# tensor4all/tensor4all-rs

Hardware: AMD Instinct MI355X
Metric: TCI2 full-sweep GF/s (d=30, chi=256 fp64) (higher is better)
Workload: dtype f64

## Files before the change

include/t4a_gpu.h:

```cpp
#ifndef T4A_GPU_H
#define T4A_GPU_H

#include <stddef.h>
#include <stdint.h>

#ifdef __cplusplus
extern "C" {
#endif
#if defined(__GNUC__)
#pragma GCC visibility push(default)
#endif

typedef int32_t t4a_gpu_status;
#define T4A_GPU_SUCCESS 0
#define T4A_GPU_NULL_POINTER (-1)
#define T4A_GPU_INVALID_ARGUMENT (-2)
#define T4A_GPU_BUFFER_TOO_SMALL (-5)
#define T4A_GPU_INTERNAL_ERROR (-6)
#define T4A_GPU_NOT_IMPLEMENTED (-7)
#define T4A_GPU_NAN_ENCOUNTERED (-8)
#define T4A_GPU_SINGULAR_MATRIX (-9)
#define T4A_GPU_NO_DEVICE (-10)
#define T4A_GPU_KERNEL_TIMEOUT (-11)
#define T4A_GPU_CALLBACK_ERROR (-12)
// ... 559 lines not shown
                                                const double* const* col_frames, size_t row_count, size_t col_count, int32_t op_kind,
                                                t4a_gpu_aci_op_fn op, void* user, size_t max_bond_dim, double tolerance,
                                                int32_t scale_tolerance, int32_t left_orthogonal, size_t* rank, size_t* row_indices,
                                                size_t* col_indices, double* pivot_errors, size_t* n_pivot_errors, double* left,
                                                double* right, double* sampled_scale, double* local_values);

t4a_gpu_status t4a_gpu_tci2_last_sweep_shapes(const t4a_gpu_tci2* h, size_t* out);
#define T4A_GPU_PROFILE_SLOTS 16
t4a_gpu_status t4a_gpu_tci2_profile_enable(t4a_gpu_tci2* h, int32_t enable);
t4a_gpu_status t4a_gpu_tci2_profile_reset(t4a_gpu_tci2* h);
t4a_gpu_status t4a_gpu_tci2_profile_get(const t4a_gpu_tci2* h, double* out );
t4a_gpu_status t4a_gpu_tci2_profile_variants(const t4a_gpu_tci2* h, double* out , size_t cap_rows, size_t* n_rows);

t4a_gpu_status t4a_gpu_tci2_chain_stats(const t4a_gpu_tci2* h, uint64_t* out );
t4a_gpu_status t4a_gpu_tci2_chain_stats_ext(const t4a_gpu_tci2* h, uint64_t* out );
t4a_gpu_status t4a_gpu_tci2_fill_stats(const t4a_gpu_tci2* h, uint64_t* out );
t4a_gpu_status t4a_gpu_tci2_rook_stats(const t4a_gpu_tci2* h, uint64_t* out );
t4a_gpu_status t4a_gpu_tci2_optimize_group(t4a_gpu_tci2* const* handles, size_t n_handles, const t4a_gpu_tci2_options* options,
                                           int32_t final_sweep1site);
t4a_gpu_status t4a_gpu_tci2_fill_site_tensors_group(t4a_gpu_tci2* const* handles, size_t n_handles);
t4a_gpu_status t4a_gpu_tci2_set_chain(t4a_gpu_tci2* h, int32_t enable, int32_t verify);
t4a_gpu_status t4a_gpu_tci2_set_callback_threads(t4a_gpu_tci2* h, size_t n_threads);
t4a_gpu_status t4a_gpu_tci2_small_stats(const t4a_gpu_tci2* h, uint64_t* out );

t4a_gpu_status t4a_gpu_fn_eval(int32_t fid, int32_t n_acc, const double* params, const uint64_t* weights,
                               const size_t* local_dims, size_t n_sites, const size_t* idx, size_t n_pts,
                               double* out);

#define T4A_GPU_GMRES_RELATIVE 0
#define T4A_GPU_GMRES_ABSOLUTE 1
// ... 234 lines not shown
```

tensor4all-rs_amd/csrc/capi.hip:

```cpp
#include "stdrng.hpp"
#include "smallrng.hpp"
#include <memory>
#include <initializer_list>
#include <mutex>

#include "patching.hpp"
#include "tci2.hpp"
#include "tree.hpp"
#include "quantics.hpp"
#include "tensorops.hpp"
#include "dense.hpp"
#include "aci.hpp"
#include "globalsearch.hpp"
#include "mpo.hpp"
#include "contraction.hpp"
#include "quanticstransform.hpp"
#include "tt_canonical.hpp"
#include "dmrg.hpp"
#include "tdvp.hpp"
#include "gse.hpp"
#include "pmpo.hpp"
#include "linsolve.hpp"
#include "swap.hpp"

// ... 1212 lines not shown
t4a_gpu_status t4a_gpu_tci2_chain_stats(const t4a_gpu_tci2* h, uint64_t* out)
{
    return guarded([&] {
        T4A_REQUIRE_PTR(h);
        T4A_REQUIRE_PTR(out);
        for (int k = 0; k < 5; ++k) out[k] = h->impl.chain_stats[k];
    });
}

t4a_gpu_status t4a_gpu_tci2_chain_stats_ext(const t4a_gpu_tci2* h, uint64_t* out)
{
    return guarded([&] {
        T4A_REQUIRE_PTR(h);
        T4A_REQUIRE_PTR(out);
        for (int k = 0; k < 4; ++k) out[k] = h->impl.chain_stats_ext[k];
    });
}

t4a_gpu_status t4a_gpu_tci2_rook_stats(const t4a_gpu_tci2* h, uint64_t* out)
{
    return guarded([&] {
        T4A_REQUIRE_PTR(h);
        T4A_REQUIRE_PTR(out);
        const RookWork& w = h->impl.rook_work();
        out[0] = w.n_device_searches;
        out[1] = w.n_device_visits;
        out[2] = w.n_host_searches;
        out[3] = w.n_host_syncs;
    });
}
// ... 4426 lines not shown
```

tensor4all-rs_amd/csrc/kernels.hpp:

```cpp
#pragma once

#include <hip/hip_runtime.h>

#include <cstddef>
#include <cstdint>

#include "../../include/t4a_testfunctions.h"

namespace t4a {

struct RrluWorkspace;

struct RrluPlan {
    int W = 1;
    int T = 256;
    int cpw = 0;
    int Mld = 0;
    size_t lds_bytes = 0;
};

RrluPlan rrlu_make_plan(int M, int N, int num_cus);

struct RrluArgs {
    const double* A;
// ... 239 lines not shown
    const int* prev_colperm;
    unsigned prev_token;
    unsigned long long* dbg;
    int defer_host_writes;
};
struct ChainWalkArgs {
    char* blocks;
    size_t block_bytes, off_piv, off_rp, off_cp, off_ts;
    double* pi;
    int n_bonds;
    int max_steps;
    double rel_tol, abs_tol;
    double* factors;
    size_t factors_stride;
    unsigned token_base;
    int timed;
    int lean_prep;
    unsigned long long* phase_ticks;
};
void chain_walk_launch(const ChainCommon& c, const FnDevice& fn, const ChainWalkArgs& w, int columns, hipStream_t stream);
void chain_indep_launch(const ChainCommon& c, int n_bonds, hipStream_t stream);
void chain_last_core_launch(const ChainCommon& c, const FnDevice& fn, double* core, int max_entries, hipStream_t stream);
void chain_prep_launch(const ChainCommon& c, const ChainPrepArgs& a, hipStream_t stream);
void chain_pi_launch(const ChainCommon& c, const FnDevice& fn, int b, int n_dep_ub, int n_ind_ub, double* out, hipStream_t stream);

constexpr int CHAIN_GROUP_MAX = 8;
struct ChainGroupSlot {
    ChainCommon c;
    FnDevice fn;
    double* pi;
// ... 336 lines not shown
```

tensor4all-rs_amd/csrc/kernels_chain.hip:

```cpp
#include "kernels.hpp"
#include "kernels_rrlu_w1_body.hpp"

namespace t4a {

namespace {

__device__ __forceinline__ const char* chain_kernarg_base()
{
#if defined(__HIP_DEVICE_COMPILE__)
    return (const char*)__builtin_amdgcn_kernarg_segment_ptr();
#else
    return nullptr;
#endif
}

constexpr int CHAIN_T = 1024;
constexpr int WALK_T = 1024;
constexpr int CHAIN_HASH = 4096;

__device__ __forceinline__ unsigned chain_hash(unsigned long long c)
{
    c ^= c >> 33;
    c *= 0xff51afd7ed558ccdull;
    c ^= c >> 29;
// ... 314 lines not shown
        if (i < nd) {
            uint64_t acc[T4A_FN_MAX_ACC] = {0, 0, 0, 0};
            for (int k = 0; k < K; ++k) acc[k] = racc[k] + ia[(size_t)j * K + k];
            out[(size_t)j * nd + i] = t4a_fn_value(fn.fid, acc, fn.params);
        }
    }
}
__global__ void __launch_bounds__(256) chain_pi_kernel(ChainCommon c, FnDevice fn, int b, double* __restrict__ out) { chain_pi_body(c, fn, b, out); }
__global__ void __launch_bounds__(256) chain_pi_group_kernel(const ChainGroupSlot* __restrict__ slots, int b)
{
    const ChainGroupSlot& s = slots[blockIdx.z];
    chain_pi_body(s.c, s.fn, b, s.pi);
}


__device__ __forceinline__ void chain_mirror_body(const ChainCommon& c, int nb)
{
    const int K = c.K;
    const size_t cap = (size_t)c.cap;
    const int gtid = (int)(blockIdx.x * blockDim.x + threadIdx.x), gsz = (int)(gridDim.x * blockDim.x);
    const int lane = (int)(threadIdx.x & 63), gwave = gtid >> 6, nwaves = gsz >> 6;
    for (int pf = gwave; pf < 2 * (nb + 1); pf += nwaves) {
        const int site = pf >> 1, fam = pf & 1;
        if ((fam == 0 && site == 0) || (fam == 1 && site == nb)) continue;
        const ChainTab& T = fam == 0 ? c.I : c.J;
        const ChainTab& Mr = fam == 0 ? c.mI : c.mJ;
        const int cnt = __hip_atomic_load(T.cnt + site, __ATOMIC_RELAXED, __HIP_MEMORY_SCOPE_AGENT);
        if (cnt < 0 || cnt > c.cap) continue;
        for (int e = lane; e < cnt * (1 + K); e += 64) {
            if (e < cnt) Mr.code[(size_t)site * cap + e] = T.code[(size_t)site * cap + e];
            else Mr.acc[(size_t)site * cap * K + (e - cnt)] = T.acc[(size_t)site * cap * K + (e - cnt)];
        }
        if (lane == 0) Mr.cnt[site] = cnt;
    }
    if (c.hdims)
        for (int e = gtid; e < nb * 4; e += gsz)
            if ((e & 3) != 3) c.hdims[e] = __hip_atomic_load(c.dims + e, __ATOMIC_RELAXED, __HIP_MEMORY_SCOPE_AGENT);
}

__global__ void __launch_bounds__(256) chain_last_core_kernel(ChainCommon c, FnDevice fn, double* __restrict__ core, int max_entries)
{
    const int site = c.n_sites - 1, K = c.K;
    const size_t cap = (size_t)c.cap;
    const int L = c.I.cnt[site], R = c.J.cnt[site], S = c.ldim[site], woff = c.woff[site];
    if (L < 1 || L > c.cap || R < 1 || R > c.cap || S < 1) return;
    const long long total = (long long)L * S * R;
    if (total > (long long)max_entries) return;
    for (long long e = (long long)blockIdx.x * blockDim.x + threadIdx.x; e < total; e += (long long)gridDim.x * blockDim.x) {
        const int l = (int)(e % L), s_ = (int)((e / L) % S), r = (int)(e / ((long long)L * S));
        uint64_t acc[T4A_FN_MAX_ACC] = {0, 0, 0, 0};
        for (int q = 0; q < K; ++q)
// ... 3 lines not shown
}

__device__ __forceinline__ void walk_phase_barrier(bool scalar_cache = true)
{
    if (scalar_cache) {
        __syncthreads();
        __builtin_amdgcn_s_dcache_inv();
        asm volatile("s_waitcnt lgkmcnt(0)" ::: "memory");
    } else {
        asm volatile("s_waitcnt lgkmcnt(0)\n\ts_barrier" ::: "memory");
    }
}
__device__ __forceinline__ int walk_div_small(int x, float rd) { return (int)(((float)x + 0.5f) * rd); }
__device__ __forceinline__ int walk_load_i32(const int* p) { return __hip_atomic_load(p, __ATOMIC_RELAXED, __HIP_MEMORY_SCOPE_AGENT); }

template <bool FORWARD>
__device__ __forceinline__ void walk_prep_wave0(const ChainCommon& c, WalkShared* ws, int b, int prev_b, unsigned prev_token, bool do_build, unsigned long long* dbg = nullptr)
{
    const unsigned long long dbg_t0 = dbg ? wall_clock64() : 0ull;
    const int lane = threadIdx.x & 63;
    const int K = c.K;
    const size_t cap = (size_t)c.cap;
    bool poison = false;
    int np = 0;
    if (prev_b >= 0) {
        const int pb = prev_b;
        const int pm = ws->dims[pb * 4], pn = ws->dims[pb * 4 + 1];
        const bool bad = ws->dims[pb * 4 + 2] != 0 || ws->prev_ires[1] != 0 || ws->prev_ires[3] != (int)prev_token || pm <= 0 || pn <= 0;
        const int r = ws->prev_ires[0];
        const int cnt = r > 0 ? r : 1;
        if (bad || cnt > c.cap || cnt > pm || cnt > pn || cnt > WALK_MAX_LIST) {
            poison = true;
        } else {
            const uint64_t* const pind_code = ws->ind_code[pb & 1];
            const uint64_t* const pind_acc = ws->ind_acc[pb & 1];
            uint64_t rc = 0, cc = 0, ra[T4A_FN_MAX_ACC] = {0, 0, 0, 0}, ca[T4A_FN_MAX_ACC] = {0, 0, 0, 0};
            if (lane < cnt) {
                const int ri = r > 0 ? ws->perm_rp[lane] : 0, ci = r > 0 ? ws->perm_cp[lane] : 0;
                rc = FORWARD ? ws->dep_code[ri] : pind_code[ri];
                cc = FORWARD ? pind_code[ci] : ws->dep_code[ci];
                for (int q = 0; q < K; ++q) {
                    ra[q] = FORWARD ? ws->dep_acc[(size_t)ri * K + q] : pind_acc[(size_t)ri * K + q];
                    ca[q] = FORWARD ? pind_acc[(size_t)ci * K + q] : ws->dep_acc[(size_t)ci * K + q];
                }
            }
            if (lane < cnt) {
                const size_t oi = (size_t)(pb + 1) * cap, oj = (size_t)pb * cap;
                c.I.code[oi + lane] = rc;
                c.J.code[oj + lane] = cc;
                ws->par_code[lane] = FORWARD ? rc : cc;
                for (int q = 0; q < K; ++q) {
                    c.I.acc[(oi + lane) * K + q] = ra[q];
                    c.J.acc[(oj + lane) * K + q] = ca[q];
                    ws->par_acc[(size_t)lane * K + q] = FORWARD ? ra[q] : ca[q];
                }
            }
            if (lane == 0) {
                c.I.cnt[pb + 1] = cnt;
// ... 114 lines not shown
    unsigned long long ph_last = ph_t0;
    auto phase = [&](int slot) {
        if (w.phase_ticks) {
            const unsigned long long now = wall_clock64();
            ph[slot] += now - ph_last;
            ph_last = now;
        }
    };
    ChainCommon cw = c;
    cw.dims = ws->dims;
    cw.hdims = nullptr;
    cw.ind_cnt = ws->ind_cnt;
    cw.dep_code = ws->dep_code;
    cw.dep_acc = ws->dep_acc;
    cw.dep_cap = WALK_MAX_LIST;
    for (int e = tid; e < nb * 4; e += (int)blockDim.x) ws->dims[e] = 0;
    for (int e = tid; e < nb; e += (int)blockDim.x) ws->ind_cnt[e] = c.ind_cnt[e];
    for (int e = tid; e <= nb; e += (int)blockDim.x) {
        ws->ldim[e] = c.ldim[e];
        ws->woff[e] = c.woff[e];
    }
    cw.ldim = ws->ldim;
    cw.woff = ws->woff;
    {
        const int nw = c.K * c.total;
        if (nw <= WALK_MAX_W) {
            for (int e = tid; e < nw; e += (int)blockDim.x) ws->w[e] = c.w[e];
            cw.w = ws->w;
        }
    }
    walk_phase_barrier();
    walk_prefetch(c, ws, FORWARD ? 0 : nb - 1, 0, (int)blockDim.x);
    walk_phase_barrier();
    for (int k = 0; k <= nb; ++k) {
        const int b = FORWARD ? k : nb - 1 - k;
        ChainPrepArgs pa;
        pa.b = b;
        pa.do_build = k < nb ? 1 : 0;
        pa.with_rowmap = 0;
        pa.prev_b = -1;
        pa.prev_iresult = nullptr;
        pa.prev_rowperm = nullptr;
        pa.prev_colperm = nullptr;
        pa.prev_token = 0u;
        pa.dbg = nullptr;
        pa.defer_host_writes = 1;
        if (k > 0) {
            pa.prev_b = FORWARD ? b - 1 : b + 1;
            pa.prev_iresult = ws->prev_ires;
            pa.prev_rowperm = ws->perm_rp;
            pa.prev_colperm = ws->perm_cp;
            pa.prev_token = w.token_base + (unsigned)(k - 1);
        }
        if (w.lean_prep) {
            if (tid < 64) walk_prep_wave0<FORWARD>(cw, ws, b, pa.prev_b, pa.prev_token, k < nb, w.phase_ticks);
        } else {
            chain_prep_body(cw, pa, w.phase_ticks, ws);
        }
        walk_phase_barrier(!w.lean_prep);
        phase(0);
        if (k == nb) break;
        const int d0 = ws->dims[b * 4], d1 = ws->dims[b * 4 + 1], poisoned = ws->dims[b * 4 + 2];
        const int nd = FORWARD ? d0 : d1, ni = FORWARD ? d1 : d0;
        const bool runs = poisoned == 0 && nd > 0 && ni > 0 && nd <= WALK_MAX_LIST && ni <= NC;
        if (runs) {
            const int K = fn.n_acc;
            const uint64_t* ia = ws->ind_acc[b & 1];
            const float rnd = 1.0f / (float)nd;
            for (int idx = tid; idx < nd * ni; idx += (int)blockDim.x) {
                const int j = walk_div_small(idx, rnd), i = idx - j * nd;
                uint64_t acc[T4A_FN_MAX_ACC] = {0, 0, 0, 0};
                for (int q = 0; q < K; ++q) acc[q] = ws->dep_acc[(size_t)i * K + q] + ia[(size_t)j * K + q];
                pi[idx] = t4a_fn_value(fn.fid, acc, fn.params);
            }
        }
        walk_phase_barrier(!w.lean_prep);
        phase(1);
        if (tid >= 64 && k + 1 < nb) walk_prefetch(c, ws, FORWARD ? b + 1 : b - 1, 64, (int)blockDim.x - 64);
        if (tid < 64) {
            int npiv = -2;
            char* blk = w.blocks + (size_t)b * w.block_bytes;
            if (runs) {
                RrluXcdArgs a = {};
                a.A = pi;
                a.Aout = FACTORS ? w.factors + (size_t)b * w.factors_stride : nullptr;
                a.urows = nullptr;
                a.M = nd;
                a.N = ni;
                a.max_steps = w.max_steps < (nd < ni ? nd : ni) ? w.max_steps : (nd < ni ? nd : ni);
                a.rel_tol = w.rel_tol;
                a.abs_tol = w.abs_tol;
                a.tie_row_major = FORWARD ? 0 : 1;
                a.out_transposed = FORWARD ? 0 : 1;
                a.W = 1;
                a.xcc = 0;
                a.ticket = nullptr;
                a.ticket_base = 0u;
                a.row_perm = FORWARD ? ws->perm_rp : ws->perm_cp;
                a.col_perm = FORWARD ? ws->perm_cp : ws->perm_rp;
                a.iresult = reinterpret_cast<int*>(blk + 16);
                a.dresult = reinterpret_cast<double*>(blk);
                a.pivot_vals = reinterpret_cast<double*>(blk + w.off_piv);
                a.keys = nullptr;
                a.salt = w.token_base + (unsigned)k;
                a.spec_frac = 0.0;
                a.stamps = nullptr;
                a.h_block = nullptr;
                a.block_u64 = 0;
                a.dims = nullptr;
                a.dims_swap = 0;
                a.rowmap = nullptr;
                a.ts_u64 = 0;
                const unsigned long long t0 = w.timed ? wall_clock64() : 0ull;
                npiv = rrlu_w1_body<NC, !FORWARD, FACTORS>(a, w1lds);
                if (npiv >= 0) {
                    int* const g_rp = reinterpret_cast<int*>(blk + w.off_rp);
                    int* const g_cp = reinterpret_cast<int*>(blk + w.off_cp);
                    if (tid < d0) g_rp[tid] = ws->perm_rp[tid];
                    if (tid < d1) g_cp[tid] = ws->perm_cp[tid];
                    if (w.timed && tid == 0) {
                        unsigned long long* ts = reinterpret_cast<unsigned long long*>(blk + w.off_ts);
                        ts[0] = t0;
                        ts[1] = wall_clock64();
                    }
                    if (tid == 0) a.iresult[3] = (int)a.salt;
                }
            }
            if (tid == 0) {
                ws->prev_ires[0] = npiv >= 0 ? npiv : 0;
                ws->prev_ires[1] = npiv >= 0 ? 0 : 1;
                ws->prev_ires[2] = 0;
                ws->prev_ires[3] = npiv >= 0 ? (int)(w.token_base + (unsigned)k) : 0;
            }
        }
        walk_phase_barrier(!w.lean_prep);
        phase(2);
    }
    for (int e = tid; e < nb * 4; e += (int)blockDim.x) c.dims[e] = ws->dims[e];
    __threadfence();
    __syncthreads();
    chain_mirror_body(c, nb);
    if (w.phase_ticks && tid == 0) {
        for (int i = 0; i < 3; ++i) w.phase_ticks[i] = ph[i];
        w.phase_ticks[3] = wall_clock64() - ph_t0;
    }
}

template <int NC, bool FORWARD, bool FACTORS> void chain_walk_launch_one(const ChainCommon& c, const FnDevice& fn, const ChainWalkArgs& w, hipStream_t stream)
{
    constexpr size_t lds = walk_lds_bytes<NC, FACTORS>();
    static std::once_flag attr_once;
    std::call_once(attr_once, [] {
        (void)hipFuncSetAttribute(reinterpret_cast<const void*>(&chain_walk_kernel<NC, FORWARD, FACTORS>), hipFuncAttributeMaxDynamicSharedMemorySize, (int)lds);
    });
    hipLaunchKernelGGL((chain_walk_kernel<NC, FORWARD, FACTORS>), dim3(1), dim3(WALK_T), lds, stream, c, fn, w);
}
// ... 63 lines not shown
```

tensor4all-rs_amd/csrc/tci2.hpp:

```cpp
#pragma once

#include <cstring>
#include <memory>
#include <vector>

#include "engine.hpp"
#include "fnsource.hpp"
#include "matrix_source.hpp"
#include "stdrng.hpp"
#include "pishard.hpp"
#include "rook.hpp"
#include "tt.hpp"

namespace t4a {

struct TCI2Options {
    double tolerance = 1e-8;
    size_t max_iter = 20;
    size_t max_bond_dim = 0;
    int pivot_search = 0;
    bool normalize_error = true;
    size_t verbosity = 0;
    size_t max_nglobal_pivot = 5;
    size_t nsearch = 5;
    int sweep_strategy = 2;
    size_t ncheck_history = 3;
    bool strictly_nested = false;
    double tol_margin_global_search = 10.0;
    bool has_seed = false;
    uint64_t seed = 0;
    size_t max_bond_dim_or_max() const { return bond_cap(max_bond_dim); }
    void validate() const;
};

struct FromTensorTrainOptions {
    double tolerance = 1e-12;
    size_t max_bond_dim = 0;
    size_t max_iter = 3;
};

struct FillZero {
    double* ptr;
    size_t count;
};
struct FillOps {
    void* flags;
    size_t flag_bytes;
    void* stage_dev;
// ... 83 lines not shown
    void fill_site_tensors();
    void fill_wait();
    void export_site_tensors_async(double* d_dst, size_t stride, hipStream_t consumer);
    void export_site_shard_async(double* d_dst, size_t stride, hipStream_t consumer);
    void import_site_shard_async(const double* d_src, size_t stride, size_t per_rank, hipStream_t producer);
    void make_canonical(double rel_tol, double abs_tol, size_t max_bond_dim);
    void invalidate_site_tensors();
    void flush_pivot_errors() { pivot_errors.clear(); }
    void mark_sets_changed()
    {
        chain_.tables_valid = false;
        chain_.digits_stale = false;
    }
    std::array<uint64_t, 5> chain_stats{{0, 0, 0, 0, 0}};
    std::array<uint64_t, 4> chain_stats_ext{{0, 0, 0, 0}};
    const uint64_t* fill_stats() const { return fill_.stats; }
    const RookWork& rook_work() const { return rook_work_; }
    bool chain_enabled = true;
    bool chain_verify = false;
    bool chain_event_timing = false;

    std::vector<double> evaluate(const uint32_t* idx, size_t n_pts);
    double sum();
    std::vector<double> site_tensor_host(size_t site, size_t dims3[3]);

    void assign_from_tensor_train(const TensorTrain& tt, const FromTensorTrainOptions& options);

    size_t n_;
    std::vector<size_t> local_dims;
    std::vector<IndexSet> i_set, j_set;
// ... 130 lines not shown
        bool in_optimize = false;
        long ext_idx = -1;
        size_t chi = 0;
        std::vector<size_t> order;
        std::vector<RrluRoute> plans;
        std::vector<unsigned> tokens;
        bool one_site = false;
        bool one_factors = false;
        double abs_tol = 0.0;
        DevBuf<double> factors, urows;
        size_t factors_stride = 0;
        bool cores_batched = false;
        bool last_core_launched = false, last_core_ok = false;
        DevBuf<unsigned long long> walk_dbg;
        bool walked = false;
        bool prep_dbg = false;
        unsigned walk_token = 1;
        RrluBlock proto;
        bool timed = false, timed_events = false;
        std::vector<hipEvent_t> t0, t1;
        bool prepared = false;
        ChainCommon common;
        std::vector<size_t> dep_ub, ind_ub;
        bool use_extras = false;
        size_t ind_cap = 0, cap_side = 0;
        double tol = 0.0;
        hipStream_t wait_stream = nullptr;
        int group_role = 0;
        hipEvent_t group_ev = nullptr;
        DevBuf<ChainGroupSlot> gslots;
// ... 39 lines not shown
```

tensor4all-rs_amd/csrc/tci2_chain.hip:

```cpp
#include "tci2.hpp"

#include <algorithm>
#include <atomic>
#include <chrono>
#include <cmath>
#include <cstdlib>

namespace t4a {

namespace {
size_t round_up_sz(size_t v, size_t m) { return (v + m - 1) / m * m; }
std::atomic<int> g_chains_inflight{0};
}
thread_local double g_chain_wait_seconds = 0.0;

bool Tci2::chain_usable(const TCI2Options& options) const
{
    static const bool off = std::getenv("T4A_NO_CHAIN") != nullptr;
    if (off || !chain_enabled || !fn_.builtin() || options.pivot_search != 0) return false;
    long double space = 1.0L;
    for (size_t d : local_dims) space *= (long double)d;
    if (space >= 9.0e18L) return false;
    for (size_t p = 0; p < n_; ++p) {
        if (i_set[p].count == 0 || j_set[p].count == 0) return false;
        if (i_set[p].count > (size_t)CHAIN_MAX_SET || j_set[p].count > (size_t)CHAIN_MAX_SET) return false;
    }
    return true;
}

// ... 195 lines not shown
    for (size_t p = 0; p < n_; ++p) {
        cI[p] = i_set[p].count;
        cJ[p] = j_set[p].count;
        if (ext) {
            eI[p] = ext->is[p].count;
            eJ[p] = ext->js[p].count;
        }
        use_extras |= eI[p] != 0 || eJ[p] != 0;
        need_cap = std::max({need_cap, cI[p], cJ[p], eI[p], eJ[p]});
    }
    std::vector<size_t> order(nb);
    for (size_t k = 0; k < nb; ++k) order[k] = forward ? k : nb - 1 - k;
    std::vector<size_t> dep_ub(nb), ind_ub(nb), lda_ub(nb, 0);
    std::vector<RrluRoute> plans(nb);
    size_t Mcap = 1, Ncap = 1, steps_cap = 1, pi_cap = 0, spec_cap = 0, dep_cap = 1, ind_cap = 1;
    for (size_t k = 0; k < nb; ++k) {
        const size_t b = order[k];
        const size_t Mub = one ? (forward ? cI[b] * local_dims[b] : cI[b + 1]) : cI[b] * local_dims[b] + eI[b + 1];
        const size_t Nub = one ? (forward ? cJ[b] : cJ[b + 1] * local_dims[b + 1]) : cJ[b + 1] * local_dims[b + 1] + eJ[b];
        const size_t rub = std::max<size_t>(std::min({Mub, Nub, chi}), 1);
        cI[b + 1] = rub;
        cJ[b] = rub;
        need_cap = std::max(need_cap, rub);
        dep_ub[b] = forward ? Mub : Nub;
        ind_ub[b] = forward ? Nub : Mub;
        if (dep_ub[b] > 65535 || ind_ub[b] > 65535 || !(plans[b] = eng.chain_route((int)dep_ub[b], (int)ind_ub[b])).ok()) {
            ++(one ? chain_stats_ext[2] : chain_stats[3]);
            return false;
        }
        Mcap = std::max(Mcap, Mub);
        Ncap = std::max(Ncap, Nub);
        dep_cap = std::max(dep_cap, dep_ub[b]);
        ind_cap = std::max(ind_cap, ind_ub[b]);
        steps_cap = std::max(steps_cap, rub);
// ... 187 lines not shown
        return k;
    };
    {
        size_t reserve_words = 0;
        const RrluRoute cr = cap_side ? eng.chain_route((int)cap_side, (int)cap_side) : RrluRoute();
        if (cr.on_xcd()) reserve_words = cr.xcd_mailbox_words();
        eng.chain_begin(plans, reserve_words);
    }
    bool counted = false;
    try {
        chain_indep_launch(c, (int)nb, st);
        unsigned* tile_counters = reinterpret_cast<unsigned*>(chain_.dims.get() + nb * 4);
        const bool solo = g_chains_inflight.fetch_add(1) == 0;
        counted = true;
        static const bool no_walk = std::getenv("T4A_NO_WALK") != nullptr;
        size_t walk_cols = 0;
        bool walk = !no_walk && !timed_events && nb <= 128;
        for (size_t b = 0; walk && b < nb; ++b) {
            walk = dep_ub[b] <= 64 && ind_ub[b] <= 32;
            walk_cols = std::max(walk_cols, ind_ub[b]);
        }
        if (walk) {
            ChainWalkArgs w;
            std::memset(&w, 0, sizeof(w));
            w.blocks = chain_.blocks.get();
            w.block_bytes = proto.bytes;
            w.off_piv = proto.off_piv;
            w.off_rp = proto.off_rp;
            w.off_cp = proto.off_cp;
            w.off_ts = proto.off_ts;
            w.pi = chain_.pi.get();
            w.n_bonds = (int)nb;
            w.max_steps = (int)std::min<size_t>(chi, 64);
            w.rel_tol = chain_.tol;
            w.abs_tol = chain_.one_site ? chain_.abs_tol : 0.0;
            w.factors = chain_.factors_stride ? chain_.factors.get() : nullptr;
            w.factors_stride = chain_.factors_stride;
            if (chain_.walk_token > 0xFFFF0000u || chain_.walk_token == 0u) chain_.walk_token = 1u;
            w.token_base = chain_.walk_token;
            chain_.walk_token += (unsigned)nb;
            w.timed = chain_.timed ? 1 : 0;
            w.lean_prep = 1;
            static const bool walk_dbg = std::getenv("T4A_WALK_DEBUG") != nullptr;
            if (walk_dbg) {
                chain_.walk_dbg.reserve(8);
                T4A_HIP(hipMemsetAsync(chain_.walk_dbg.get(), 0, 8 * sizeof(unsigned long long), st));
                w.phase_ticks = chain_.walk_dbg.get();
            }
            chain_.walked = true;
            for (size_t k = 0; k < nb; ++k) tokens[order[k]] = w.token_base + (unsigned)k;
            chain_walk_launch(c, fn_.dev, w, (int)walk_cols, st);
            ++chain_stats_ext[0];
        }
        static const bool want_prep_dbg = std::getenv("T4A_PREP_DEBUG") != nullptr;
        unsigned long long* prep_dbg = nullptr;
        if (want_prep_dbg && !walk) {
            chain_.walk_dbg.reserve(8);
            T4A_HIP(hipMemsetAsync(chain_.walk_dbg.get(), 0, 8 * sizeof(unsigned long long), st));
            prep_dbg = chain_.walk_dbg.get();
            chain_.prep_dbg = true;
        }
        bool spec_pending = false;
        for (size_t k = 0; !walk && k < nb; ++k) {
            const size_t b = order[k];
            const RrluRoute& pl = plans[b];
            const bool fused = pl.fused;
            const bool spec_here = spec_pending && !fused;
            const RrluBlock blk = block_of(b);
            ChainPrepArgs pa;
            std::memset(&pa, 0, sizeof(pa));
            pa.b = (int)b;
            pa.do_build = 1;
            pa.dbg = prep_dbg;
            pa.defer_host_writes = 0;
            pa.with_rowmap = spec_here ? 1 : 0;
            pa.prev_b = -1;
            if (k > 0) {
                const size_t pb = order[k - 1];
                const RrluBlock pblk = block_of(pb);
                pa.prev_b = (int)pb;
                pa.prev_iresult = pblk.iresult();
                pa.prev_rowperm = pblk.row_perm();
                pa.prev_colperm = pblk.col_perm();
                pa.prev_token = tokens[pb];
            }
            chain_prep_launch(c, pa, st);
            if (!fused && !spec_here) chain_pi_launch(c, fn_.dev, (int)b, (int)dep_ub[b], (int)ind_ub[b], chain_.pi.get(), st);
            XcdSpecArgs sp;
            std::memset(&sp, 0, sizeof(sp));
            spec_pending = false;
            if (solo && k + 1 < nb && pl.on_xcd()) {
                const size_t nx = order[k + 1];
                if (!plans[nx].fused) {
                    const size_t site = forward ? nx : nx + 1;
                    const ChainTab& H = forward ? c.HI : c.HJ;
                    const size_t hsite = forward ? nx + 1 : nx;
                    sp.out = chain_.spec[(k + 1) & 1].get();
                    sp.dep_acc = c.dep_acc;
                    sp.w_site = c.w + fn_.offset[site];
                    sp.ext_acc = H.acc + hsite * cap * K;
                    sp.ext_cnt = use_extras ? H.cnt + hsite : nullptr;
                    sp.ind_acc = c.ind_acc + nx * ind_cap * K;
                    sp.ind_cnt = c.ind_cnt + nx;
                    sp.tile_counter = tile_counters + nx;
                    sp.total = (int)fn_.total;
                    sp.d = (int)local_dims[site];
// ... 1 lines not shown
                    spec_pending = true;
                }
            }
            FusedPi fp;
            fp.fn = fn_.dev;
            fp.d_rowacc = c.dep_acc;
            fp.d_colacc = c.ind_acc + b * ind_cap * K;
            fp.host_resident = false;
            const double* A = fused ? nullptr : (spec_here ? chain_.spec[k & 1].get() : chain_.pi.get());
            if (timed_events) T4A_HIP(hipEventRecord(chain_.t0[b], st));
            tokens[b] = eng.chain_rrlu(pl, forward, A, spec_here ? c.rowmap : nullptr, fused ? &fp : nullptr, c.dims + b * 4, chi, chain_.tol,
                                       chain_.one_site ? chain_.abs_tol : 0.0, blk, spec_pending ? &sp : nullptr,
                                       chain_.factors_stride ? chain_.factors.get() + b * chain_.factors_stride : nullptr, chain_.urows.get());
            if (timed_events) T4A_HIP(hipEventRecord(chain_.t1[b], st));
        }
        if (!walk) {
            const size_t pb = order[nb - 1];
            const RrluBlock pblk = block_of(pb);
            ChainPrepArgs pa;
            std::memset(&pa, 0, sizeof(pa));
            pa.do_build = 0;
            pa.defer_host_writes = 0;
            pa.prev_b = (int)pb;
            pa.prev_iresult = pblk.iresult();
            pa.prev_rowperm = pblk.row_perm();
            pa.prev_colperm = pblk.col_perm();
            pa.prev_token = tokens[pb];
            chain_prep_launch(c, pa, st);
        }
        chain_.cores_batched = false;
        if (chain_.one_site && chain_.factors_stride && forward && nb <= (size_t)LUCI_LEFT_CORES_MAX_JOBS) {
// ... 154 lines not shown
            T4A_HIP(hipMemcpyAsync(h->chain_.hblocks.get(), h->chain_.blocks.get(), nb * h->chain_.proto.bytes, hipMemcpyDeviceToHost, st));
        T4A_HIP(hipGetLastError());
    } catch (...) {
        (void)hipStreamSynchronize(st);
        if (locked) lead->eng.chain_end();
        for (size_t i = 0; i < nh; ++i) {
            if (counted[i]) g_chains_inflight.fetch_sub(1);
            hs[i]->chain_.prepared = false;
            hs[i]->chain_.tables_valid = false;
            hs[i]->chain_.snap_serial[0] = hs[i]->chain_.snap_serial[1] = ~0ull;
        }
        throw;
    }
    for (Tci2* h : hs) {
        h->chain_.plans = gplans;
        h->chain_.inflight = true;
        h->chain_.wait_stream = st;
        h->chain_.group_role = h == lead ? 1 : 2;
    }
}

void Tci2::chain_abort() noexcept
{
    if (chain_.prepared) {
        chain_.snap_serial[0] = chain_.snap_serial[1] = ~0ull;
        chain_.tables_valid = false;
    }
    chain_.prepared = false;
    chain_.walked = false;
    if (!chain_.inflight) return;
// ... 213 lines not shown
                        same = dev[(size_t)side * fam + p * cap + k] == m.code[p * cap + k];
                        for (size_t q = 0; same && q < K; ++q)
                            same = dev[(size_t)side * fam + n_ * cap + (p * cap + k) * K + q] == m.acc[(p * cap + k) * K + q];
                    }
                    if (!same)
                        throw Error(T4A_GPU_INTERNAL_ERROR, std::string("bond chain: device table ") + (side == 0 ? "I_" : "J_") + std::to_string(p) +
                                                                " differs from its host mirror");
                }
        }
        return;
    }
    ++(chain_.one_site ? chain_stats_ext[3] : chain_stats[2]);
    sync_digits();
    chain_.tables_valid = false;
    if (failed_timeout) {
        const RrluKind kind = chain_.plans[chain_.order[(size_t)failed_k]].kind;
        if (kind == RrluKind::SingleXcd || kind == RrluKind::MultiXcd) xcd_disable();
    }
    prep_.valid = false;
    prefetch_.wanted = false;
    prefetch_.fill_site = -1;
    invalidate_fill_cache();
    std::vector<IndexSet> no_i(n_), no_j(n_);
    for (size_t p = 0; p < n_; ++p) {
        no_i[p].width = p;
        no_j[p].width = n_ - p - 1;
    }
    const std::vector<IndexSet>* xi = &no_i;
    const std::vector<IndexSet>* xj = &no_j;
    if (chain_.ext_idx >= 0) {
        HistEntry& e = history[(size_t)chain_.ext_idx];
        hist_digits(e);
// ... 14 lines not shown
```

tensor4all-rs_amd/python/t4a_amd/__init__.py:

```python
import ctypes
import os

import numpy as np

from .functions import (FnSpec, quantics_trig_exp, quantics_osc2d, lorentz, linear_sum,
                        FN_MAX_PARAMS)

_HERE = os.path.dirname(os.path.abspath(__file__))
LIB_PATH = os.environ.get("T4A_GPU_LIB") or os.path.normpath(os.path.join(_HERE, "..", "..", "lib", "libt4a_gpu.so"))

if not os.path.exists(LIB_PATH):
    raise ImportError(f"{LIB_PATH} not found: build it with `python tensor4all-rs_amd/build.py` "
                      "(the MI355X backend has no CPU fallback)")

_lib = ctypes.CDLL(LIB_PATH)

c_size_t = ctypes.c_size_t
c_double = ctypes.c_double
c_int32 = ctypes.c_int32
c_void_p = ctypes.c_void_p

SUCCESS = 0
NULL_POINTER = -1
INVALID_ARGUMENT = -2
# ... 783 lines not shown
        return {"device_searches": int(out[0]), "device_visits": int(out[1]), "host_searches": int(out[2]), "host_syncs": int(out[3])}

    def fill_stats(self):
        out = (ctypes.c_uint64 * 3)()
        _check(_lib.t4a_gpu_tci2_fill_stats(self._h, out))
        return {"fills": int(out[0]), "graph_replays": int(out[1]), "graph_captures": int(out[2])}

    def chain_stats(self):
        out = np.zeros(5, dtype=np.uint64)
        _check(_lib.t4a_gpu_tci2_chain_stats(self._h, _p(out)))
        ext = np.zeros(4, dtype=np.uint64)
        _check(_lib.t4a_gpu_tci2_chain_stats_ext(self._h, _p(ext)))
        return dict(half_sweeps=int(out[0]), bonds=int(out[1]), fell_back=int(out[2]), not_eligible=int(out[3]),
                    group_half_sweeps=int(out[4]), walked_sweeps=int(ext[0]), one_site_sweeps=int(ext[1]),
                    one_site_not_eligible=int(ext[2]), one_site_fell_back=int(ext[3]))


def optimize_group(tcis, options, final_sweep1site=True):
    o = options.to_c()
    arr = (c_void_p * len(tcis))(*[t._h for t in tcis])
    _check(_lib.t4a_gpu_tci2_optimize_group(arr, c_size_t(len(tcis)), ctypes.byref(o), c_int32(1 if final_sweep1site else 0)))


def fill_site_tensors_group(tcis):
    arr = (c_void_p * len(tcis))(*[t._h for t in tcis])
    _check(_lib.t4a_gpu_tci2_fill_site_tensors_group(arr, c_size_t(len(tcis))))


def crossinterpolate2(f, local_dims, initial_pivots, options):
    options.to_c()
# ... 1241 lines not shown
```

Measured before the change: 340.3.

## Walk eligible bond segments in a single kernel when the whole chain cannot be walked

Before this change the single-kernel chain walk ran only when every bond in the half-sweep met the small dependent/independent bound limits. Otherwise each bond fell back to per-bond launches. The new code splits the sweep order into runs of walkable and non-walkable bonds. It launches the walk kernel for each walkable run, seeding its first prep from the previous block's global results, and it writes the dependent list back to global memory for the bonds that follow. It also tightens the two-site M/N upper bounds using the full left/right index space sizes, which can make more bonds fit the walk limits. The trade-off is more complex handoff state between walked and non-walked segments, plus a risk of correctness issues at segment boundaries.

```diff
diff --git a/include/t4a_gpu.h b/include/t4a_gpu.h
--- a/include/t4a_gpu.h
+++ b/include/t4a_gpu.h
@@ -597,6 +597,9 @@
 
 t4a_gpu_status t4a_gpu_tci2_chain_stats(const t4a_gpu_tci2* h, uint64_t* out );
 t4a_gpu_status t4a_gpu_tci2_chain_stats_ext(const t4a_gpu_tci2* h, uint64_t* out );
+t4a_gpu_status t4a_gpu_tci2_chain_segments(const t4a_gpu_tci2* h, uint64_t* out );
+t4a_gpu_status t4a_gpu_tci2_chain_plan_segments(const size_t* dep_ub, const size_t* ind_ub, const size_t* order, size_t n_bonds, size_t capacity,
+                                                size_t* first, size_t* count, int32_t* walked, size_t* n_segments);
 t4a_gpu_status t4a_gpu_tci2_fill_stats(const t4a_gpu_tci2* h, uint64_t* out );
 t4a_gpu_status t4a_gpu_tci2_rook_stats(const t4a_gpu_tci2* h, uint64_t* out );
 t4a_gpu_status t4a_gpu_tci2_optimize_group(t4a_gpu_tci2* const* handles, size_t n_handles, const t4a_gpu_tci2_options* options,
diff --git a/tensor4all-rs_amd/csrc/capi.hip b/tensor4all-rs_amd/csrc/capi.hip
--- a/tensor4all-rs_amd/csrc/capi.hip
+++ b/tensor4all-rs_amd/csrc/capi.hip
@@ -1250,6 +1250,42 @@
         T4A_REQUIRE_PTR(h);
         T4A_REQUIRE_PTR(out);
         for (int k = 0; k < 4; ++k) out[k] = h->impl.chain_stats_ext[k];
+    });
+}
+
+t4a_gpu_status t4a_gpu_tci2_chain_segments(const t4a_gpu_tci2* h, uint64_t* out)
+{
+    return guarded([&] {
+        T4A_REQUIRE_PTR(h);
+        T4A_REQUIRE_PTR(out);
+        for (int k = 0; k < 2; ++k) out[k] = h->impl.chain_segments[k];
+    });
+}
+
+t4a_gpu_status t4a_gpu_tci2_chain_plan_segments(const size_t* dep_ub, const size_t* ind_ub, const size_t* order, size_t n_bonds, size_t capacity,
+                                                size_t* first, size_t* count, int32_t* walked, size_t* n_segments)
+{
+    return guarded([&] {
+        T4A_REQUIRE_PTR(n_segments);
+        if (n_bonds > 0) {
+            T4A_REQUIRE_PTR(dep_ub);
+            T4A_REQUIRE_PTR(ind_ub);
+            T4A_REQUIRE_PTR(order);
+        }
+        for (size_t k = 0; k < n_bonds; ++k)
+            if (order[k] >= n_bonds) throw t4a::Error(T4A_GPU_INVALID_ARGUMENT, "chain_plan_segments: order[" + std::to_string(k) + "] is not a bond of the chain");
+        const std::vector<t4a::ChainSegment> segs = t4a::chain_plan_segments(dep_ub, ind_ub, order, n_bonds);
+        *n_segments = segs.size();
+        if (!first && !count && !walked) return;
+        T4A_REQUIRE_PTR(first);
+        T4A_REQUIRE_PTR(count);
+        T4A_REQUIRE_PTR(walked);
+        if (capacity < segs.size()) throw t4a::Error(T4A_GPU_BUFFER_TOO_SMALL, "chain_plan_segments: " + std::to_string(segs.size()) + " segments, room for " + std::to_string(capacity));
+        for (size_t s = 0; s < segs.size(); ++s) {
+            first[s] = segs[s].first;
+            count[s] = segs[s].count;
+            walked[s] = segs[s].walked ? 1 : 0;
+        }
     });
 }
 
diff --git a/tensor4all-rs_amd/csrc/kernels.hpp b/tensor4all-rs_amd/csrc/kernels.hpp
--- a/tensor4all-rs_amd/csrc/kernels.hpp
+++ b/tensor4all-rs_amd/csrc/kernels.hpp
@@ -277,6 +277,11 @@
     double* factors;
     size_t factors_stride;
     unsigned token_base;
+    int k_first, k_count;
+    const int* prev_iresult;
+    const int* prev_rowperm;
+    const int* prev_colperm;
+    unsigned prev_token;
     int timed;
     int lean_prep;
     unsigned long long* phase_ticks;
diff --git a/tensor4all-rs_amd/csrc/kernels_chain.hip b/tensor4all-rs_amd/csrc/kernels_chain.hip
--- a/tensor4all-rs_amd/csrc/kernels_chain.hip
+++ b/tensor4all-rs_amd/csrc/kernels_chain.hip
@@ -352,15 +352,14 @@
 }
 
 
-__device__ __forceinline__ void chain_mirror_body(const ChainCommon& c, int nb)
+__device__ __forceinline__ void chain_mirror_body(const ChainCommon& c, int g_lo, int g_hi, int b_lo, int b_hi)
 {
     const int K = c.K;
     const size_t cap = (size_t)c.cap;
     const int gtid = (int)(blockIdx.x * blockDim.x + threadIdx.x), gsz = (int)(gridDim.x * blockDim.x);
     const int lane = (int)(threadIdx.x & 63), gwave = gtid >> 6, nwaves = gsz >> 6;
-    for (int pf = gwave; pf < 2 * (nb + 1); pf += nwaves) {
-        const int site = pf >> 1, fam = pf & 1;
-        if ((fam == 0 && site == 0) || (fam == 1 && site == nb)) continue;
+    for (int pf = 2 * g_lo + gwave; pf < 2 * g_hi; pf += nwaves) {
+        const int fam = pf & 1, site = (pf >> 1) + (fam == 0 ? 1 : 0);
         const ChainTab& T = fam == 0 ? c.I : c.J;
         const ChainTab& Mr = fam == 0 ? c.mI : c.mJ;
         const int cnt = __hip_atomic_load(T.cnt + site, __ATOMIC_RELAXED, __HIP_MEMORY_SCOPE_AGENT);
@@ -372,7 +371,7 @@
         if (lane == 0) Mr.cnt[site] = cnt;
     }
     if (c.hdims)
-        for (int e = gtid; e < nb * 4; e += gsz)
+        for (int e = b_lo * 4 + gtid; e < b_hi * 4; e += gsz)
             if ((e & 3) != 3) c.hdims[e] = __hip_atomic_load(c.dims + e, __ATOMIC_RELAXED, __HIP_MEMORY_SCOPE_AGENT);
 }
 
@@ -406,8 +405,15 @@
 __device__ __forceinline__ int walk_div_small(int x, float rd) { return (int)(((float)x + 0.5f) * rd); }
 __device__ __forceinline__ int walk_load_i32(const int* p) { return __hip_atomic_load(p, __ATOMIC_RELAXED, __HIP_MEMORY_SCOPE_AGENT); }
 
-template <bool FORWARD>
-__device__ __forceinline__ void walk_prep_wave0(const ChainCommon& c, WalkShared* ws, int b, int prev_b, unsigned prev_token, bool do_build, unsigned long long* dbg = nullptr)
+struct WalkPrevGlobal {
+    const int* dims;
+    const int *iresult, *rowperm, *colperm;
+    const uint64_t *dep_code, *dep_acc;
+    const uint64_t *ind_code, *ind_acc;
+};
+template <bool FORWARD, bool PREV_GLOBAL = false>
+__device__ __forceinline__ void walk_prep_wave0(const ChainCommon& c, WalkShared* ws, int b, int prev_b, unsigned prev_token, bool do_build, unsigned long long* dbg = nullptr,
+                                                const WalkPrevGlobal* g = nullptr)
 {
     const unsigned long long dbg_t0 = dbg ? wall_clock64() : 0ull;
     const int lane = threadIdx.x & 63;
@@ -417,23 +423,29 @@
     int np = 0;
     if (prev_b >= 0) {
         const int pb = prev_b;
-        const int pm = ws->dims[pb * 4], pn = ws->dims[pb * 4 + 1];
-        const bool bad = ws->dims[pb * 4 + 2] != 0 || ws->prev_ires[1] != 0 || ws->prev_ires[3] != (int)prev_token || pm <= 0 || pn <= 0;
-        const int r = ws->prev_ires[0];
+        const int* const pdims = PREV_GLOBAL ? g->dims : ws->dims + pb * 4;
+        const int* const pires = PREV_GLOBAL ? g->iresult : ws->prev_ires;
+        const int pm = pdims[0], pn = pdims[1];
+        const bool bad = pdims[2] != 0 || pires[1] != 0 || pires[3] != (int)prev_token || pm <= 0 || pn <= 0;
+        const int r = pires[0];
         const int cnt = r > 0 ? r : 1;
         if (bad || cnt > c.cap || cnt > pm || cnt > pn || cnt > WALK_MAX_LIST) {
             poison = true;
         } else {
-            const uint64_t* const pind_code = ws->ind_code[pb & 1];
-            const uint64_t* const pind_acc = ws->ind_acc[pb & 1];
+            const uint64_t* const pind_code = PREV_GLOBAL ? g->ind_code : ws->ind_code[pb & 1];
+            const uint64_t* const pind_acc = PREV_GLOBAL ? g->ind_acc : ws->ind_acc[pb & 1];
+            const uint64_t* const pdep_code = PREV_GLOBAL ? g->dep_code : ws->dep_code;
+            const uint64_t* const pdep_acc = PREV_GLOBAL ? g->dep_acc : ws->dep_acc;
+            const int* const prp = PREV_GLOBAL ? g->rowperm : ws->perm_rp;
+            const int* const pcp = PREV_GLOBAL ? g->colperm : ws->perm_cp;
             uint64_t rc = 0, cc = 0, ra[T4A_FN_MAX_ACC] = {0, 0, 0, 0}, ca[T4A_FN_MAX_ACC] = {0, 0, 0, 0};
             if (lane < cnt) {
-                const int ri = r > 0 ? ws->perm_rp[lane] : 0, ci = r > 0 ? ws->perm_cp[lane] : 0;
-                rc = FORWARD ? ws->dep_code[ri] : pind_code[ri];
-                cc = FORWARD ? pind_code[ci] : ws->dep_code[ci];
+                const int ri = r > 0 ? prp[lane] : 0, ci = r > 0 ? pcp[lane] : 0;
+                rc = FORWARD ? pdep_code[ri] : pind_code[ri];
+                cc = FORWARD ? pind_code[ci] : pdep_code[ci];
                 for (int q = 0; q < K; ++q) {
-                    ra[q] = FORWARD ? ws->dep_acc[(size_t)ri * K + q] : pind_acc[(size_t)ri * K + q];
-                    ca[q] = FORWARD ? pind_acc[(size_t)ci * K + q] : ws->dep_acc[(size_t)ci * K + q];
+                    ra[q] = FORWARD ? pdep_acc[(size_t)ri * K + q] : pind_acc[(size_t)ri * K + q];
+                    ca[q] = FORWARD ? pind_acc[(size_t)ci * K + q] : pdep_acc[(size_t)ci * K + q];
                 }
             }
             if (lane < cnt) {
@@ -578,9 +590,13 @@
     cw.dep_code = ws->dep_code;
     cw.dep_acc = ws->dep_acc;
     cw.dep_cap = WALK_MAX_LIST;
-    for (int e = tid; e < nb * 4; e += (int)blockDim.x) ws->dims[e] = 0;
-    for (int e = tid; e < nb; e += (int)blockDim.x) ws->ind_cnt[e] = c.ind_cnt[e];
-    for (int e = tid; e <= nb; e += (int)blockDim.x) {
+    const int k0 = w.k_first, k1 = w.k_first + w.k_count;
+    const bool behind = k0 > 0;
+    const bool ends = k1 == nb;
+    const int b_lo = FORWARD ? k0 : nb - k1, b_hi = FORWARD ? k1 : nb - k0;
+    for (int e = b_lo * 4 + tid; e < b_hi * 4; e += (int)blockDim.x) ws->dims[e] = 0;
+    for (int e = b_lo + tid; e < b_hi; e += (int)blockDim.x) ws->ind_cnt[e] = c.ind_cnt[e];
+    for (int e = b_lo + tid; e <= b_hi; e += (int)blockDim.x) {
         ws->ldim[e] = c.ldim[e];
         ws->woff[e] = c.woff[e];
     }
@@ -594,13 +610,26 @@
         }
     }
     walk_phase_barrier();
-    walk_prefetch(c, ws, FORWARD ? 0 : nb - 1, 0, (int)blockDim.x);
+    walk_prefetch(c, ws, FORWARD ? k0 : nb - 1 - k0, 0, (int)blockDim.x);
     walk_phase_barrier();
-    for (int k = 0; k <= nb; ++k) {
+    WalkPrevGlobal pg = {};
+    if (behind) {
+        const int pb = FORWARD ? k0 - 1 : nb - k0;
+        pg.dims = c.dims + (size_t)pb * 4;
+        pg.iresult = w.prev_iresult;
+        pg.rowperm = w.prev_rowperm;
+        pg.colperm = w.prev_colperm;
+        pg.dep_code = c.dep_code;
+        pg.dep_acc = c.dep_acc;
+        pg.ind_code = c.ind_code + (size_t)pb * c.ind_cap;
+        pg.ind_acc = c.ind_acc + (size_t)pb * c.ind_cap * c.K;
+    }
+    const int k_end = ends ? k1 : k1 - 1;
+    for (int k = k0; k <= k_end; ++k) {
         const int b = FORWARD ? k : nb - 1 - k;
         ChainPrepArgs pa;
         pa.b = b;
-        pa.do_build = k < nb ? 1 : 0;
+        pa.do_build = k < k1 ? 1 : 0;
         pa.with_rowmap = 0;
         pa.prev_b = -1;
         pa.prev_iresult = nullptr;
@@ -609,21 +638,23 @@
         pa.prev_token = 0u;
         pa.dbg = nullptr;
         pa.defer_host_writes = 1;
-        if (k > 0) {
+        if (k > k0) {
             pa.prev_b = FORWARD ? b - 1 : b + 1;
             pa.prev_iresult = ws->prev_ires;
             pa.prev_rowperm = ws->perm_rp;
             pa.prev_colperm = ws->perm_cp;
-            pa.prev_token = w.token_base + (unsigned)(k - 1);
-        }
-        if (w.lean_prep) {
-            if (tid < 64) walk_prep_wave0<FORWARD>(cw, ws, b, pa.prev_b, pa.prev_token, k < nb, w.phase_ticks);
+            pa.prev_token = w.token_base + (unsigned)(k - k0 - 1);
+        }
+        if (k == k0 && behind) {
+            if (tid < 64) walk_prep_wave0<FORWARD, true>(cw, ws, b, FORWARD ? b - 1 : b + 1, w.prev_token, true, w.phase_ticks, &pg);
+        } else if (w.lean_prep) {
+            if (tid < 64) walk_prep_wave0<FORWARD>(cw, ws, b, pa.prev_b, pa.prev_token, k < k1, w.phase_ticks);
         } else {
             chain_prep_body(cw, pa, w.phase_ticks, ws);
         }
         walk_phase_barrier(!w.lean_prep);
         phase(0);
-        if (k == nb) break;
+        if (k == k1) break;
         const int d0 = ws->dims[b * 4], d1 = ws->dims[b * 4 + 1], poisoned = ws->dims[b * 4 + 2];
         const int nd = FORWARD ? d0 : d1, ni = FORWARD ? d1 : d0;
         const bool runs = poisoned == 0 && nd > 0 && ni > 0 && nd <= WALK_MAX_LIST && ni <= NC;
@@ -640,7 +671,7 @@
         }
         walk_phase_barrier(!w.lean_prep);
         phase(1);
-        if (tid >= 64 && k + 1 < nb) walk_prefetch(c, ws, FORWARD ? b + 1 : b - 1, 64, (int)blockDim.x - 64);
+        if (tid >= 64 && k + 1 < k1) walk_prefetch(c, ws, FORWARD ? b + 1 : b - 1, 64, (int)blockDim.x - 64);
         if (tid < 64) {
             int npiv = -2;
             char* blk = w.blocks + (size_t)b * w.block_bytes;
@@ -666,7 +697,7 @@
                 a.dresult = reinterpret_cast<double*>(blk);
                 a.pivot_vals = reinterpret_cast<double*>(blk + w.off_piv);
                 a.keys = nullptr;
-                a.salt = w.token_base + (unsigned)k;
+                a.salt = w.token_base + (unsigned)(k - k0);
                 a.spec_frac = 0.0;
                 a.stamps = nullptr;
                 a.h_block = nullptr;
@@ -694,16 +725,27 @@
                 ws->prev_ires[0] = npiv >= 0 ? npiv : 0;
                 ws->prev_ires[1] = npiv >= 0 ? 0 : 1;
                 ws->prev_ires[2] = 0;
-                ws->prev_ires[3] = npiv >= 0 ? (int)(w.token_base + (unsigned)k) : 0;
+                ws->prev_ires[3] = npiv >= 0 ? (int)(w.token_base + (unsigned)(k - k0)) : 0;
             }
         }
         walk_phase_barrier(!w.lean_prep);
         phase(2);
     }
-    for (int e = tid; e < nb * 4; e += (int)blockDim.x) c.dims[e] = ws->dims[e];
+    for (int e = b_lo * 4 + tid; e < b_hi * 4; e += (int)blockDim.x) c.dims[e] = ws->dims[e];
+    if (!ends) {
+        const int bl = FORWARD ? k1 - 1 : nb - k1;
+        int nd = ws->dims[bl * 4 + 2] != 0 ? 0 : ws->dims[bl * 4 + (FORWARD ? 0 : 1)];
+        nd = nd < 0 ? 0 : (nd > WALK_MAX_LIST ? WALK_MAX_LIST : nd);
+        if (nd > c.dep_cap) nd = 0;
+        for (int e = tid; e < nd * (1 + c.K); e += (int)blockDim.x) {
+            if (e < nd) c.dep_code[e] = ws->dep_code[e];
+            else c.dep_acc[e - nd] = ws->dep_acc[e - nd];
+        }
+    }
     __threadfence();
     __syncthreads();
-    chain_mirror_body(c, nb);
+    const int gk0 = behind ? k0 - 1 : k0, gk1 = ends ? k1 : k1 - 1;
+    chain_mirror_body(c, FORWARD ? gk0 : nb - gk1, FORWARD ? gk1 : nb - gk0, b_lo, b_hi);
     if (w.phase_ticks && tid == 0) {
         for (int i = 0; i < 3; ++i) w.phase_ticks[i] = ph[i];
         w.phase_ticks[3] = wall_clock64() - ph_t0;
diff --git a/tensor4all-rs_amd/csrc/tci2.hpp b/tensor4all-rs_amd/csrc/tci2.hpp
--- a/tensor4all-rs_amd/csrc/tci2.hpp
+++ b/tensor4all-rs_amd/csrc/tci2.hpp
@@ -32,6 +32,13 @@
     size_t max_bond_dim_or_max() const { return bond_cap(max_bond_dim); }
     void validate() const;
 };
+
+constexpr size_t CHAIN_WALK_MAX_DEP = 64, CHAIN_WALK_MAX_IND = 32;
+struct ChainSegment {
+    size_t first, count;
+    bool walked;
+};
+std::vector<ChainSegment> chain_plan_segments(const size_t* dep_ub, const size_t* ind_ub, const size_t* order, size_t n_bonds);
 
 struct FromTensorTrainOptions {
     double tolerance = 1e-12;
@@ -145,6 +152,7 @@
     }
     std::array<uint64_t, 5> chain_stats{{0, 0, 0, 0, 0}};
     std::array<uint64_t, 4> chain_stats_ext{{0, 0, 0, 0}};
+    std::array<uint64_t, 2> chain_segments{{0, 0}};
     const uint64_t* fill_stats() const { return fill_.stats; }
     const RookWork& rook_work() const { return rook_work_; }
     bool chain_enabled = true;
@@ -305,6 +313,7 @@
         bool last_core_launched = false, last_core_ok = false;
         DevBuf<unsigned long long> walk_dbg;
         bool walked = false;
+        std::vector<char> seg_walked;
         bool prep_dbg = false;
         unsigned walk_token = 1;
         RrluBlock proto;
diff --git a/tensor4all-rs_amd/csrc/tci2_chain.hip b/tensor4all-rs_amd/csrc/tci2_chain.hip
--- a/tensor4all-rs_amd/csrc/tci2_chain.hip
+++ b/tensor4all-rs_amd/csrc/tci2_chain.hip
@@ -13,6 +13,20 @@
 std::atomic<int> g_chains_inflight{0};
 }
 thread_local double g_chain_wait_seconds = 0.0;
+
+std::vector<ChainSegment> chain_plan_segments(const size_t* dep_ub, const size_t* ind_ub, const size_t* order, size_t n_bonds)
+{
+    std::vector<ChainSegment> segs;
+    for (size_t k = 0; k < n_bonds; ++k) {
+        const size_t b = order[k];
+        const bool walked = dep_ub[b] <= CHAIN_WALK_MAX_DEP && ind_ub[b] <= CHAIN_WALK_MAX_IND;
+        if (!segs.empty() && segs.back().walked == walked)
+            ++segs.back().count;
+        else
+            segs.push_back(ChainSegment{k, 1, walked});
+    }
+    return segs;
+}
 
 bool Tci2::chain_usable(const TCI2Options& options) const
 {
@@ -238,10 +252,18 @@
     std::vector<size_t> dep_ub(nb), ind_ub(nb), lda_ub(nb, 0);
     std::vector<RrluRoute> plans(nb);
     size_t Mcap = 1, Ncap = 1, steps_cap = 1, pi_cap = 0, spec_cap = 0, dep_cap = 1, ind_cap = 1;
+    std::vector<size_t> space_l(nb, 1), space_r(nb, 1);
+    if (!one) {
+        const size_t big = (size_t)1 << 40;
+        size_t acc = 1;
+        for (size_t b = 0; b < nb; ++b) space_l[b] = acc = std::min(big, acc * local_dims[b]);
+        acc = 1;
+        for (size_t b = nb; b-- > 0;) space_r[b] = acc = std::min(big, acc * local_dims[b + 1]);
+    }
     for (size_t k = 0; k < nb; ++k) {
         const size_t b = order[k];
-        const size_t Mub = one ? (forward ? cI[b] * local_dims[b] : cI[b + 1]) : cI[b] * local_dims[b] + eI[b + 1];
-        const size_t Nub = one ? (forward ? cJ[b] : cJ[b + 1] * local_dims[b + 1]) : cJ[b + 1] * local_dims[b + 1] + eJ[b];
+        const size_t Mub = one ? (forward ? cI[b] * local_dims[b] : cI[b + 1]) : std::min(cI[b] * local_dims[b] + eI[b + 1], space_l[b]);
+        const size_t Nub = one ? (forward ? cJ[b] : cJ[b + 1] * local_dims[b + 1]) : std::min(cJ[b + 1] * local_dims[b + 1] + eJ[b], space_r[b]);
         const size_t rub = std::max<size_t>(std::min({Mub, Nub, chi}), 1);
         cI[b + 1] = rub;
         cJ[b] = rub;
@@ -459,13 +481,26 @@
         const bool solo = g_chains_inflight.fetch_add(1) == 0;
         counted = true;
         static const bool no_walk = std::getenv("T4A_NO_WALK") != nullptr;
-        size_t walk_cols = 0;
-        bool walk = !no_walk && !timed_events && nb <= 128;
-        for (size_t b = 0; walk && b < nb; ++b) {
-            walk = dep_ub[b] <= 64 && ind_ub[b] <= 32;
-            walk_cols = std::max(walk_cols, ind_ub[b]);
-        }
-        if (walk) {
+        const bool may_walk = !no_walk && !timed_events && nb <= 128;
+        std::vector<ChainSegment> segs;
+        if (may_walk) segs = chain_plan_segments(dep_ub.data(), ind_ub.data(), order.data(), nb);
+        const bool walk = may_walk && (nb == 0 || (segs.size() == 1 && segs[0].walked));
+        std::vector<char> walked_k(nb, walk ? 1 : 0);
+        if (may_walk && !walk && !chain_.one_site)
+            for (const ChainSegment& s : segs)
+                for (size_t k = s.first; s.walked && k < s.first + s.count; ++k) walked_k[k] = 1;
+        chain_.seg_walked.assign(nb, 0);
+        for (size_t k = 0; k < nb; ++k) chain_.seg_walked[order[k]] = walked_k[k];
+        static const bool plan_dbg = std::getenv("T4A_CHAIN_DEBUG") != nullptr;
+        if (plan_dbg) {
+            std::fprintf(stderr, "[t4a chain] %s half-sweep, %zu bonds, dependent x independent bounds in sweep order (w: walked):", forward ? "forward" : "backward", nb);
+            for (size_t k = 0; k < nb; ++k) std::fprintf(stderr, " %zux%zu%s", dep_ub[order[k]], ind_ub[order[k]], walked_k[k] ? "w" : "");
+            std::fprintf(stderr, "\n");
+        }
+        auto launch_walk = [&](size_t first, size_t count) {
+            size_t walk_cols = 0;
+            for (size_t k = first; k < first + count; ++k) walk_cols = std::max(walk_cols, ind_ub[order[k]]);
+            const bool whole = count == nb;
             ChainWalkArgs w;
             std::memset(&w, 0, sizeof(w));
             w.blocks = chain_.blocks.get();
@@ -483,20 +518,36 @@
             w.factors_stride = chain_.factors_stride;
             if (chain_.walk_token > 0xFFFF0000u || chain_.walk_token == 0u) chain_.walk_token = 1u;
             w.token_base = chain_.walk_token;
-            chain_.walk_token += (unsigned)nb;
+            chain_.walk_token += (unsigned)count;
+            w.k_first = (int)first;
+            w.k_count = (int)count;
+            if (first > 0) {
+                const size_t pb = order[first - 1];
+                const RrluBlock pblk = block_of(pb);
+                w.prev_iresult = pblk.iresult();
+                w.prev_rowperm = pblk.row_perm();
+                w.prev_colperm = pblk.col_perm();
+                w.prev_token = tokens[pb];
+            }
             w.timed = chain_.timed ? 1 : 0;
             w.lean_prep = 1;
             static const bool walk_dbg = std::getenv("T4A_WALK_DEBUG") != nullptr;
-            if (walk_dbg) {
+            if (walk_dbg && whole) {
                 chain_.walk_dbg.reserve(8);
                 T4A_HIP(hipMemsetAsync(chain_.walk_dbg.get(), 0, 8 * sizeof(unsigned long long), st));
                 w.phase_ticks = chain_.walk_dbg.get();
             }
-            chain_.walked = true;
-            for (size_t k = 0; k < nb; ++k) tokens[order[k]] = w.token_base + (unsigned)k;
+            for (size_t k = 0; k < count; ++k) tokens[order[first + k]] = w.token_base + (unsigned)k;
             chain_walk_launch(c, fn_.dev, w, (int)walk_cols, st);
-            ++chain_stats_ext[0];
-        }
+            if (whole) {
+                chain_.walked = true;
+                ++chain_stats_ext[0];
+            } else {
+                ++chain_segments[0];
+                chain_segments[1] += count;
+            }
+        };
+        if (walk) launch_walk(0, nb);
         static const bool want_prep_dbg = std::getenv("T4A_PREP_DEBUG") != nullptr;
         unsigned long long* prep_dbg = nullptr;
         if (want_prep_dbg && !walk) {
@@ -507,6 +558,14 @@
         }
         bool spec_pending = false;
         for (size_t k = 0; !walk && k < nb; ++k) {
+            if (walked_k[k]) {
+                size_t count = 1;
+                while (k + count < nb && walked_k[k + count]) ++count;
+                launch_walk(k, count);
+                k += count - 1;
+                spec_pending = false;
+                continue;
+            }
             const size_t b = order[k];
             const RrluRoute& pl = plans[b];
             const bool fused = pl.fused;
@@ -534,7 +593,7 @@
             XcdSpecArgs sp;
             std::memset(&sp, 0, sizeof(sp));
             spec_pending = false;
-            if (solo && k + 1 < nb && pl.on_xcd()) {
+            if (solo && k + 1 < nb && !walked_k[k + 1] && pl.on_xcd()) {
                 const size_t nx = order[k + 1];
                 if (!plans[nx].fused) {
                     const size_t site = forward ? nx : nx + 1;
@@ -566,7 +625,7 @@
                                        chain_.factors_stride ? chain_.factors.get() + b * chain_.factors_stride : nullptr, chain_.urows.get());
             if (timed_events) T4A_HIP(hipEventRecord(chain_.t1[b], st));
         }
-        if (!walk) {
+        if (nb > 0 && !walked_k[nb - 1]) {
             const size_t pb = order[nb - 1];
             const RrluBlock pblk = block_of(pb);
             ChainPrepArgs pa;
@@ -751,6 +810,7 @@
     }
     for (Tci2* h : hs) {
         h->chain_.plans = gplans;
+        h->chain_.seg_walked.clear();
         h->chain_.inflight = true;
         h->chain_.wait_stream = st;
         h->chain_.group_role = h == lead ? 1 : 2;
@@ -994,8 +1054,10 @@
     sync_digits();
     chain_.tables_valid = false;
     if (failed_timeout) {
-        const RrluKind kind = chain_.plans[chain_.order[(size_t)failed_k]].kind;
-        if (kind == RrluKind::SingleXcd || kind == RrluKind::MultiXcd) xcd_disable();
+        const size_t fb = chain_.order[(size_t)failed_k];
+        const RrluKind kind = chain_.plans[fb].kind;
+        const bool in_walk = fb < chain_.seg_walked.size() && chain_.seg_walked[fb];
+        if (!in_walk && (kind == RrluKind::SingleXcd || kind == RrluKind::MultiXcd)) xcd_disable();
     }
     prep_.valid = false;
     prefetch_.wanted = false;
diff --git a/tensor4all-rs_amd/python/t4a_amd/__init__.py b/tensor4all-rs_amd/python/t4a_amd/__init__.py
--- a/tensor4all-rs_amd/python/t4a_amd/__init__.py
+++ b/tensor4all-rs_amd/python/t4a_amd/__init__.py
@@ -821,6 +821,27 @@
         return dict(half_sweeps=int(out[0]), bonds=int(out[1]), fell_back=int(out[2]), not_eligible=int(out[3]),
                     group_half_sweeps=int(out[4]), walked_sweeps=int(ext[0]), one_site_sweeps=int(ext[1]),
                     one_site_not_eligible=int(ext[2]), one_site_fell_back=int(ext[3]))
+
+    def chain_segments(self):
+        out = np.zeros(2, dtype=np.uint64)
+        _check(_lib.t4a_gpu_tci2_chain_segments(self._h, _p(out)))
+        return dict(segments=int(out[0]), bonds=int(out[1]))
+
+
+def chain_plan_segments(dep_ub, ind_ub, order):
+    dep = np.ascontiguousarray(dep_ub, dtype=np.uintp)
+    ind = np.ascontiguousarray(ind_ub, dtype=np.uintp)
+    order = np.ascontiguousarray(order, dtype=np.uintp)
+    nb = int(order.size)
+    if dep.size != nb or ind.size != nb:
+        raise T4aError(INVALID_ARGUMENT, "chain_plan_segments: dep_ub, ind_ub and order have one entry per bond")
+    ptr = (lambda a: _p(a) if nb else None)
+    n = ctypes.c_size_t(0)
+    _check(_lib.t4a_gpu_tci2_chain_plan_segments(ptr(dep), ptr(ind), ptr(order), ctypes.c_size_t(nb), ctypes.c_size_t(0), None, None, None, ctypes.byref(n)))
+    k = n.value
+    first, count, walked = np.zeros(max(k, 1), dtype=np.uintp), np.zeros(max(k, 1), dtype=np.uintp), np.zeros(max(k, 1), dtype=np.int32)
+    _check(_lib.t4a_gpu_tci2_chain_plan_segments(ptr(dep), ptr(ind), ptr(order), ctypes.c_size_t(nb), ctypes.c_size_t(k), _p(first), _p(count), _p(walked), ctypes.byref(n)))
+    return [(int(first[s]), int(count[s]), bool(walked[s])) for s in range(k)]
 
 
 def optimize_group(tcis, options, final_sweep1site=True):
```

Result: faster. 347.2, median of 6 (+2.0%).
